# rajan-dubey8/camouflage-multimodal

Measured on AMD Instinct MI355X. Metric: images/sec fwd+bwd (fusion model train step: fwd + loss + bwd + clip + AdamW), higher is better.
Workload: dtype bf16; 1 GPU; BASELINE configs[1] on the path that exists (SURVEY 8d): cross-attention fusion model, packed variable-Nr minibatch (Nr ~ real 303..530 histogram, mean 483), Nk=13 real KG rows, train mode dropout 0.3, random-init weights; batch_per_gpu=16, global_batch=16, rg_dim=128, hidden_dim=256, num_heads=8, parallelism=dp1, precision=bf16 MFMA operands, fp32 accumulate/optimizer

## Files before the change

camouflage_multimodal_amd/csrc/fused_rows.hip:

```cpp
#include "fused_rows.h"
#include "shadow_inl.h"
#include "gemm.h"
#include "mfma_inl.h"

namespace {

template <int NT, int KS, bool W_IS_A, int DEPTH, bool USE_ROT = true>
struct Stage {
  static constexpr int TOTAL = NT * KS;
  static constexpr int D = DEPTH < TOTAL ? DEPTH : TOTAL;
  static_assert(!USE_ROT || (KS & (KS - 1)) == 0, "rotated k order: power-of-two k steps");
  u32x4 buf[D];
  const u32x4* wp; int rot;
  __device__ __forceinline__ int keff(int ks) const { return USE_ROT ? ((ks + rot) & (KS - 1)) : ks; }
  __device__ __forceinline__ const u32x4* wptr(int i) const { return wp + 64 * (keff(i / NT) * NT + (i % NT)); }
  __device__ __forceinline__ void prefetch(const u32x4* __restrict__ wp_, int rot_) {
    wp = wp_; rot = rot_;
#pragma unroll
    for (int i = 0; i < D; ++i) buf[i] = *wptr(i);
  }
  __device__ __forceinline__ void run(const char* act, f32x16 (&acc)[NT]) {
    run_f([&](int ks) { return *reinterpret_cast<const bf16x8*>(act + 32 * ks); }, acc);
  }
  template <class F>
// ... 31 lines not shown
__global__ __launch_bounds__(256) void shadow_kernel(const ShadowBatch sb, int total_chunks) {
  const int gid = blockIdx.x * 256 + threadIdx.x;
  for (int zi = 0; zi < sb.nzero; ++zi) {
    u32x4* z = static_cast<u32x4*>(sb.zero_ptr[zi]);
    const size_t n16 = sb.zero_bytes[zi] >> 4;
    for (size_t i = gid; i < n16; i += (size_t)gridDim.x * 256) z[i] = u32x4{0u, 0u, 0u, 0u};
  }
  if (gid >= total_chunks) return;
  int ji = 0;
#pragma unroll
  for (int i = 1; i < SHADOW_MAXJ; ++i)
    if (i < sb.n && gid >= sb.j[i].chunk_begin) ji = i;
  shadow_chunk(sb.j[ji], gid - sb.j[ji].chunk_begin);
}

constexpr int F_BUFR = 32 * PX, F_BUFQ = F_BUFR + 32 * PR, F_LDS = F_BUFQ + 32 * PQ;

template <int DEPTH, bool ROT>
__global__ __launch_bounds__(256, 2) void front_kernel(const FrontArgs a) {
  extern __shared__ __attribute__((aligned(16))) char smem[];
  const FrontStream& S = a.s[(int)blockIdx.x >= a.s[1].tile_begin ? 1 : 0];
  const int tid = threadIdx.x, lane = tid & 63, l31 = lane & 31, h = lane >> 5;
  const int w = __builtin_amdgcn_readfirstlane(tid >> 6);
  const int row0 = ((int)blockIdx.x - S.tile_begin) * 32;
  const int nrows = min(32, S.M - row0);
  char* bufX = smem; char* bufR = smem + F_BUFR; char* bufQ = smem + F_BUFQ;
  const int rot = ROT ? (int)(blockIdx.x >> 3) : 0;
  stamp(a.stamps, 0);
  Stage<2, 8, true, DEPTH> st0;
  st0.prefetch(reinterpret_cast<const u32x4*>(S.W0) + (size_t)w * (8 * 2 * 64) + lane, rot);
  {
    const int r = tid >> 3, c = tid & 7;
    const float4* src = reinterpret_cast<const float4*>(S.X + (size_t)(row0 + min(r, nrows - 1)) * 128 + 16 * c);
    float4 v0 = src[0], v1 = src[1], v2 = src[2], v3 = src[3];
    if (r >= nrows) { v0 = v1 = v2 = v3 = make_float4(0.f, 0.f, 0.f, 0.f); }
    *reinterpret_cast<u32x4*>(bufX + r * PX + 32 * c) = u32x4{pack2(v0.x, v0.y), pack2(v0.z, v0.w), pack2(v1.x, v1.y), pack2(v1.z, v1.w)};
    *reinterpret_cast<u32x4*>(bufX + r * PX + 32 * c + 16) = u32x4{pack2(v2.x, v2.y), pack2(v2.z, v2.w), pack2(v3.x, v3.y), pack2(v3.z, v3.w)};
  }
  __syncthreads();
  Stage<6, 16, true, DEPTH> st1;
  {
    f32x16 acc[2] = {zero16(), zero16()};
    st0.run(bufX + l31 * PX + 16 * h, acc);
    st1.prefetch(reinterpret_cast<const u32x4*>(S.W1) + (size_t)w * (16 * 6 * 64) + lane, rot);
#pragma unroll
    for (int t = 0; t < 2; ++t)
#pragma unroll
      for (int g = 0; g < 4; ++g) {
        const int c0 = 64 * w + 32 * t + 8 * g + 4 * h;
        const float4 bv = *reinterpret_cast<const float4*>(S.b0 + c0);
        *reinterpret_cast<u32x2*>(bufR + l31 * PR + 2 * c0) =
            u32x2{pack2(acc[t][4 * g] + bv.x, acc[t][4 * g + 1] + bv.y), pack2(acc[t][4 * g + 2] + bv.z, acc[t][4 * g + 3] + bv.w)};
      }
  }
  __syncthreads();
  stamp(a.stamps, 1);
  {
    f32x16 acc[6];
#pragma unroll
    for (int t = 0; t < 6; ++t) acc[t] = zero16();
    st1.run(bufR + l31 * PR + 16 * h, acc);
#pragma unroll
    for (int t = 0; t < 6; ++t) {
      const int tg = 6 * w + t;
      const float* bias = tg < 8 ? S.bq + 32 * tg : S.bkv + 32 * (tg - 8);
      const float sc = tg < 8 ? a.qscale : 1.0f;
#pragma unroll
      for (int g = 0; g < 4; ++g) {
        const int c = 8 * g + 4 * h;
        const float4 bv = *reinterpret_cast<const float4*>(bias + c);
        *reinterpret_cast<u32x2*>(bufQ + l31 * PQ + 2 * (32 * tg + c)) =
            u32x2{pack2((acc[t][4 * g] + bv.x) * sc, (acc[t][4 * g + 1] + bv.y) * sc),
                  pack2((acc[t][4 * g + 2] + bv.z) * sc, (acc[t][4 * g + 3] + bv.w) * sc)};
      }
    }
  }
  __syncthreads();
  stamp(a.stamps, 2);
  copy_out<5>(bufQ, PQ, 0, S.Q16, 256, row0, nrows);
  copy_out<6>(bufQ, PQ, 512, S.KV16, 512, row0, nrows);
  copy_out<5>(bufR, PR, 0, S.R16, 256, row0, nrows);
  if (a.save) copy_out<4>(bufX, PX, 0, S.X16, 128, row0, nrows);
  for (int zi = 0; zi < a.nzero; ++zi) {
    u32x4* z = static_cast<u32x4*>(a.zero_ptr[zi]);
    const unsigned n16 = a.zero_bytes[zi] >> 4;
    for (unsigned i = blockIdx.x * 256 + tid; i < n16; i += gridDim.x * 256) z[i] = u32x4{0u, 0u, 0u, 0u};
  }
  stamp(a.stamps, 3);
}

constexpr int PK = 528;
constexpr int PVC = 192;
constexpr int PT = 260;
constexpr int B_VS = 16 * PK;
template <int OCC> struct BackL;
template <> struct BackL<2> { static constexpr int XH = 0, O = 32 * PT * 4, Y = O + 32 * PR, RED = Y + 32 * PR, LDS = RED + 1024; };
template <> struct BackL<3> { static constexpr int Y = 0, XH = 32 * PR, O = 2 * 32 * PR, RED = O + 32 * PR, LDS = RED + 1024; };
constexpr int B_LDS = BackL<2>::LDS;
static_assert(BackL<3>::O >= 4 * 32 * 192 && BackL<3>::O >= 8448 + 9216 && BackL<2>::O >= 4 * 32 * 192, "attention scratch inside region A");

__device__ __forceinline__ void attn_rg_tile(const BackArgs& a, char* smem, char* bufO, int b, size_t row0, int nrows, int w, int lane) {
  const int tid = threadIdx.x, l31 = lane & 31, h = lane >> 5, Nk = a.Nk;
  char* Ks = smem; char* Vs = smem + B_VS;
  for (int c = tid; c < 16 * 64; c += 256) {
    const int j = c >> 6, ch = c & 63;
    u32x4 v = u32x4{0u, 0u, 0u, 0u};
    if (j < Nk) v = *reinterpret_cast<const u32x4*>(a.KV16 + ((size_t)b * Nk + j) * 512 + 8 * ch);
    if (ch < 32) *reinterpret_cast<u32x4*>(Ks + j * PK + 16 * ch) = v;
    else         *reinterpret_cast<u32x4*>(Vs + j * PV + 16 * (ch - 32)) = v;
  }
  const us16* qrow = a.Q16 + (row0 + min(l31, nrows - 1)) * 256 + 64 * w + 8 * h;
  bf16x8 qf[2][2];
#pragma unroll
  for (int hd = 0; hd < 2; ++hd)
#pragma unroll
    for (int s = 0; s < 2; ++s) qf[hd][s] = as_frag(*reinterpret_cast<const u32x4*>(qrow + 32 * hd + 16 * s));
  __syncthreads();
  const bool dodrop = a.drop.p > 0.f;
  const int q4 = (lane >> 2) & 3, p4 = lane & 3, g1 = (lane >> 4) & 1;
#pragma unroll
  for (int hd = 0; hd < 2; ++hd) {
    const int head = 2 * w + hd;
// ... 201 lines not shown
  const int w = __builtin_amdgcn_readfirstlane(tid >> 6);
  const int nkg = a.B * a.max_splits;
  const int vid = (int)blockIdx.x < a.lead_tiles ? nkg + (int)blockIdx.x : ((int)blockIdx.x < a.lead_tiles + nkg ? (int)blockIdx.x - a.lead_tiles : (int)blockIdx.x);
  const bool kg = vid < nkg;
  int rot = ROT ? (int)(blockIdx.x >> 3) : 0;
  using L = BackL<OCC>;
  char* bufO = smem + L::O; char* bufY = smem + L::Y;
  float* red = reinterpret_cast<float*>(smem + L::RED);
  float* tile32 = reinterpret_cast<float*>(smem);
  int b; size_t rowg0; int nrows; float inv_n;
  stamp(a.stamps, 0);
  const BackStream& S = a.s[kg ? 1 : 0];
  Stage<2, 16, true, DEPTH> sto;
  Stage<4, 16, false, DEPTH> stf;
  if (!kg) sto.prefetch(reinterpret_cast<const u32x4*>(S.Wo) + (size_t)w * (16 * 2 * 64) + lane, rot);
  if (kg) {
    b = vid / a.max_splits;
    const int sp = vid - b * a.max_splits;
    if (ROT) rot = b;
    const int nsplit = (a.off[b + 1] - a.off[b] + SPLIT_ROWS - 1) / SPLIT_ROWS;
    if (sp >= nsplit) return;
    attn_kg_split(a, smem, b, sp, w, lane);
    stamp(a.stamps, 4);
    asm volatile("s_waitcnt vmcnt(0)" ::: "memory");
    __syncthreads();
    int* flag = reinterpret_cast<int*>(red);
    if (tid == 0) flag[0] = __hip_atomic_fetch_add(a.tickets + b, 1, __ATOMIC_RELAXED, __HIP_MEMORY_SCOPE_AGENT);
    __syncthreads();
    stamp(a.stamps, 5);
    if (flag[0] != nsplit - 1) return;
    if (tid == 0) {
      __builtin_amdgcn_fence(__ATOMIC_ACQUIRE, "agent");
      asm volatile("s_waitcnt vmcnt(0)" ::: "memory");
    }
    for (int c = tid; c < 32 * PR / 16; c += 256) reinterpret_cast<u32x4*>(bufO)[c] = u32x4{0u, 0u, 0u, 0u};
    __syncthreads();
    sto.prefetch(reinterpret_cast<const u32x4*>(S.Wo) + (size_t)w * (16 * 2 * 64) + lane, rot);
    attn_kg_combine(a, smem, bufO, b, nsplit);
    stamp(a.stamps, 6);
    rowg0 = (size_t)b * a.Nk; nrows = a.Nk; inv_n = 1.0f / (float)a.Nk;
  } else {
    const int4 td = a.tile_desc[vid - nkg];
    if (td.x < 0) return;
    b = td.x; rowg0 = td.y; nrows = td.z; inv_n = __int_as_float(td.w);
    attn_rg_tile(a, smem, bufO, b, rowg0, nrows, w, lane);
  }
  __syncthreads();
  stamp(a.stamps, 1);

  const size_t rrow = rowg0 + min(l31, nrows - 1);
  float u[32];
  float rstd_keep = 0.f;
  {
    f32x16 acc[2] = {zero16(), zero16()};
    sto.run(bufO + l31 * PR + 16 * h, acc);
    stf.prefetch(reinterpret_cast<const u32x4*>(S.W1) + (size_t)w * (16 * 4 * 64) + lane, rot);
    float part = 0.f;
#pragma unroll
    for (int t = 0; t < 2; ++t)
#pragma unroll
      for (int g = 0; g < 4; ++g) {
        const int c0 = 64 * w + 32 * t + 8 * g + 4 * h;
        const float4 bv = *reinterpret_cast<const float4*>(S.bo + c0);
        const u32x2 rv = *reinterpret_cast<const u32x2*>(S.R16 + rrow * 256 + c0);
        float* o = u + 16 * t + 4 * g;
        o[0] = acc[t][4 * g] + bv.x + bf_lo(rv.x); o[1] = acc[t][4 * g + 1] + bv.y + bf_hi(rv.x);
        o[2] = acc[t][4 * g + 2] + bv.z + bf_lo(rv.y); o[3] = acc[t][4 * g + 3] + bv.w + bf_hi(rv.y);
        part += (o[0] + o[1]) + (o[2] + o[3]);
      }
    auto row_total = [&](float p, int slot) {
      p += __shfl_xor(p, 32, 64);
      if (h == 0) red[slot * 128 + w * 32 + l31] = p;
      __syncthreads();
      return (red[slot * 128 + l31] + red[slot * 128 + 32 + l31]) + (red[slot * 128 + 64 + l31] + red[slot * 128 + 96 + l31]);
    };
    const float mean = row_total(part, 0) * (1.0f / 256.0f);
    float sq = 0.f;
#pragma unroll
    for (int i = 0; i < 32; ++i) { u[i] -= mean; sq = fmaf(u[i], u[i], sq); }
    const float rstd = 1.0f / sqrtf(row_total(sq, 1) * (1.0f / 256.0f) + 1e-5f);
    rstd_keep = rstd;
    const bool rok = l31 < nrows;
#pragma unroll
    for (int t = 0; t < 2; ++t) {
      float ys[16];
#pragma unroll
      for (int g = 0; g < 4; ++g) {
        const int c0 = 64 * w + 32 * t + 8 * g + 4 * h;
        const float4 gm = *reinterpret_cast<const float4*>(S.ln_g + c0), bt = *reinterpret_cast<const float4*>(S.ln_b + c0);
        float* o = u + 16 * t + 4 * g;
        const float x0 = o[0] * rstd, x1 = o[1] * rstd, x2 = o[2] * rstd, x3 = o[3] * rstd;
        const float4 y = make_float4(x0 * gm.x + bt.x, x1 * gm.y + bt.y, x2 * gm.z + bt.z, x3 * gm.w + bt.w);
        *reinterpret_cast<u32x2*>(bufY + l31 * PR + 2 * c0) = u32x2{pack2(y.x, y.y), pack2(y.z, y.w)};
        if constexpr (OCC == 3) {
          ys[4 * g] = rok ? y.x : 0.f; ys[4 * g + 1] = rok ? y.y : 0.f; ys[4 * g + 2] = rok ? y.z : 0.f; ys[4 * g + 3] = rok ? y.w : 0.f;
          if (a.save) *reinterpret_cast<u32x2*>(smem + L::XH + l31 * PR + 2 * c0) = u32x2{pack2(x0, x1), pack2(x2, x3)};
        } else {
          *reinterpret_cast<float4*>(tile32 + l31 * PT + c0) = y;
          o[0] = x0; o[1] = x1; o[2] = x2; o[3] = x3;
        }
      }
      if constexpr (OCC == 2) continue;
#pragma unroll
      for (int st = 0; st < 4; ++st) {
// ... 3 lines not shown
        for (int i = 0; i < n; ++i) {
          const float send = up ? ys[i] : ys[i + n];
          const float keep = up ? ys[i + n] : ys[i];
          ys[i] = keep + __shfl_xor(send, m, 64);
        }
      }
      const float tot = ys[0] + __shfl_xor(ys[0], 1, 64);
      if ((l31 & 1) == 0) {
        const int i16 = (l31 >> 1) & 15;
        atomicAdd(S.Ymean + (size_t)b * 256 + 64 * w + 32 * t + 8 * (i16 >> 2) + 4 * h + (i16 & 3), tot * inv_n);
      }
    }
  }
  __syncthreads();
  stamp(a.stamps, 2);
  if constexpr (OCC == 2) {
    float sum = 0.f;
    for (int r = 0; r < nrows; ++r) sum += tile32[r * PT + tid];
    atomicAdd(S.Ymean + (size_t)b * 256 + tid, sum * inv_n);
  }

  {
    f32x16 acc[4] = {zero16(), zero16(), zero16(), zero16()};
    stf.run(bufY + l31 * PR + 16 * h, acc);
    const bool dodrop = a.drop.p > 0.f;
#pragma unroll
    for (int t = 0; t < 4; ++t) {
      const int f = 128 * w + 32 * t + l31;
      const float bias = S.b1[f];
      float colsum = 0.f;
      uint32_t wlo = 0u, whi = 0u;
#pragma unroll
      for (int i = 0; i < 16; ++i) {
        if (8 * (i >> 2) >= nrows) continue;
        const int row = acc_row(i, h);
        float v = fmaxf(acc[t][i] + bias, 0.f);
        if (dodrop) v *= drop_mult(a.drop, S.site_ffn, (uint32_t)(rowg0 + row) * 512u + (uint32_t)f);
        if (row >= nrows) v = 0.f;
        colsum += v;
        if (a.save) {
          const unsigned long long bal = __ballot(v > 0.f);
          SET_LANE(wlo, (uint32_t)bal, i); SET_LANE(whi, (uint32_t)(bal >> 32), i);
        }
      }
// ... 17 lines not shown
        for (int g = 0; g < 4; ++g) {
          const float* o = u + 16 * t + 4 * g;
          *reinterpret_cast<u32x2*>(bufXH + l31 * PR + 2 * (64 * w + 32 * t + 8 * g + 4 * h)) = u32x2{pack2(o[0], o[1]), pack2(o[2], o[3])};
        }
      __syncthreads();
    }
    copy_out<5>(bufXH, PR, 0, S.XH16, 256, rowg0, nrows);
    copy_out<5>(bufO, PR, 0, S.O16, 256, rowg0, nrows);
    copy_out<5>(bufY, PR, 0, S.Y16, 256, rowg0, nrows);
  }
  stamp(a.stamps, 3);
}


constexpr int W_GTAB = 0, W_BUFDU = 1024, W_KS = W_BUFDU + 32 * PR, W_VS = W_KS + 16 * PK, W_BUFDO = W_VS + 16 * PK,
              W_IMGS = W_BUFDO + 32 * PR, W_RED = W_IMGS + 16384, W_LDS = W_RED + 1024;
static_assert(32 * PR + 16384 == 32 * PT * 4, "the fp32 column-sum tile aliases [bufdO | images]");

__device__ __forceinline__ void tail_wg_tile(const TailWgArgs& g, int tile, float* dys, unsigned long long* stamps) {
  stamp(stamps, 0);
  int pi = 0;
  for (int i = 1; i < g.n; ++i) if (tile >= g.p[i].tile_begin) pi = i;
  const TailWgProd& P = g.p[pi];
  const int tid = threadIdx.x, B = g.B, ncb = P.cols >> 8, lt = tile - P.tile_begin, rb = lt / ncb;
  const int r0 = 16 * rb, c = 256 * (lt - rb * ncb) + tid;
  float xv[16], acc[16];
#pragma unroll
  for (int b = 0; b < 16; ++b) xv[b] = b < B ? P.x[(size_t)b * P.ld_x + c] : 0.f;
  const float dv = tid < B * 16 ? P.dy[(size_t)(tid >> 4) * P.ld_dy + r0 + (tid & 15)] : 0.f;
#pragma unroll
  for (int r = 0; r < 16; ++r) acc[r] = P.dW[(size_t)(r0 + r) * P.cols + c];
// ... 83 lines not shown
    const int4 td = a.tile_desc[blockIdx.x];
    if (td.x < 0) return;
    b = td.x; rowg0 = td.y; nrows = td.z; inv_n = __int_as_float(td.w);
  }
  const Bwd1Stream& S = a.s[kg ? 1 : 0];
  us16* gtab = reinterpret_cast<us16*>(smem + W_GTAB);
  char* bufdU = smem + W_BUFDU; char* bufQ = bufdU;
  char* Ks = smem + W_KS; char* Vs = smem + W_VS; char* bufdO = smem + W_BUFDO; char* imgs = smem + W_IMGS + w * 4096;
  float* red = reinterpret_cast<float*>(smem + W_RED);
  float* tile32 = reinterpret_cast<float*>(smem + W_BUFDO);
  stamp(a.stamps, 0);
  Stage<2, 32, true, DEPTH, false> st1;
  st1.prefetch(reinterpret_cast<const u32x4*>(S.W1T) + (size_t)w * (32 * 2 * 64) + lane, 0);
  const size_t vrow = rowg0 + min(l31, nrows - 1);
  const bool rok = l31 < nrows;
  {
    const float gs = inv_n * a.drop.scale;
    for (int f = tid; f < 512; f += 256) gtab[f] = f2bf(S.dHm[(size_t)b * S.ld_dHm + f] * gs);
  }
  u32x4 mw[4];
#pragma unroll
  for (int i = 0; i < 4; ++i) mw[i] = reinterpret_cast<const u32x4*>(S.mask + vrow * 16)[i];
  u32x4 qreg[4];
  if (!kg) {
#pragma unroll
    for (int i = 0; i < 4; ++i) {
      const int id = tid + 256 * i;
      qreg[i] = *reinterpret_cast<const u32x4*>(a.Q16 + (rowg0 + min(id >> 5, nrows - 1)) * 256 + 8 * (id & 31));
    }
    for (int c = tid; c < 16 * 64; c += 256) {
      const int j = c >> 6, ch = c & 63;
      u32x4 v = u32x4{0u, 0u, 0u, 0u};
      if (j < a.Nk) v = *reinterpret_cast<const u32x4*>(a.KV16 + ((size_t)b * a.Nk + j) * 512 + 8 * ch);
      if (ch < 32) *reinterpret_cast<u32x4*>(Ks + j * PK + 16 * ch) = v;
      else         *reinterpret_cast<u32x4*>(Vs + j * PK + 16 * (ch - 32)) = v;
    }
  }
  __syncthreads();
  Stage<2, 16, true, DEPTH> st2;
  f32x16 acc1[2] = {zero16(), zero16()};
  st1.run_f([&](int ks) {
    const uint32_t word = mw[ks >> 3][(ks >> 1) & 3];
    const uint32_t bits = (word >> (16 * (ks & 1))) >> (8 * h);
    const u32x4 g = *reinterpret_cast<const u32x4*>(smem + W_GTAB + 2 * (16 * ks + 8 * h));
    u32x4 fr;
#pragma unroll
    for (int d = 0; d < 4; ++d)
      fr[d] = (((bits >> (2 * d)) & 1u) ? (g[d] & 0xFFFFu) : 0u) | (((bits >> (2 * d + 1)) & 1u) ? (g[d] & 0xFFFF0000u) : 0u);
    return as_frag(fr);
  }, acc1);
  st2.prefetch(reinterpret_cast<const u32x4*>(S.WoT) + (size_t)w * (16 * 2 * 64) + lane, rot);
  stamp(a.stamps, 1);
  {
    float gg[32], xh[32];
    float s1 = 0.f, s2 = 0.f;
#pragma unroll
    for (int t = 0; t < 2; ++t)
#pragma unroll
      for (int g = 0; g < 4; ++g) {
        const int c0 = 64 * w + 32 * t + 8 * g + 4 * h;
        const float4 dc = *reinterpret_cast<const float4*>(S.dcomb + (size_t)b * S.ld_dcomb + c0);
        const float4 gm = *reinterpret_cast<const float4*>(S.ln_g + c0);
        const u32x2 xv = *reinterpret_cast<const u32x2*>(S.XH16 + vrow * 256 + c0);
        float* G = gg + 16 * t + 4 * g; float* X = xh + 16 * t + 4 * g;
        X[0] = bf_lo(xv.x); X[1] = bf_hi(xv.x); X[2] = bf_lo(xv.y); X[3] = bf_hi(xv.y);
        const float d0 = fmaf(dc.x, inv_n, acc1[t][4 * g]), d1 = fmaf(dc.y, inv_n, acc1[t][4 * g + 1]);
        const float d2 = fmaf(dc.z, inv_n, acc1[t][4 * g + 2]), d3 = fmaf(dc.w, inv_n, acc1[t][4 * g + 3]);
        *reinterpret_cast<float4*>(tile32 + l31 * PT + c0) = make_float4(d0 * X[0], d1 * X[1], d2 * X[2], d3 * X[3]);
        acc1[t][4 * g] = d0; acc1[t][4 * g + 1] = d1; acc1[t][4 * g + 2] = d2; acc1[t][4 * g + 3] = d3;
        G[0] = d0 * gm.x; G[1] = d1 * gm.y; G[2] = d2 * gm.z; G[3] = d3 * gm.w;
#pragma unroll
        for (int i = 0; i < 4; ++i) { s1 += G[i]; s2 = fmaf(G[i], X[i], s2); }
      }
    auto row_total = [&](float p, int slot) {
      p += __shfl_xor(p, 32, 64);
      if (h == 0) red[slot * 128 + w * 32 + l31] = p;
      __syncthreads();
      return (red[slot * 128 + l31] + red[slot * 128 + 32 + l31]) + (red[slot * 128 + 64 + l31] + red[slot * 128 + 96 + l31]);
    };
    const float m1 = row_total(s1, 0) * (1.0f / 256.0f);
    const float m2 = row_total(s2, 1) * (1.0f / 256.0f);
    {
      float sum = 0.f;
      for (int r = 0; r < nrows; ++r) sum += tile32[r * PT + tid];
      if (a.slabs & 1) a.slabLN[(size_t)blockIdx.x * 512 + tid] = sum;
      else atomicAdd(S.dgamma + tid, sum);
    }
    const float rstd = S.rstd[vrow];
#pragma unroll
    for (int t = 0; t < 2; ++t)
#pragma unroll
      for (int g = 0; g < 4; ++g) {
        const int c0 = 64 * w + 32 * t + 8 * g + 4 * h;
        const float* G = gg + 16 * t + 4 * g; const float* X = xh + 16 * t + 4 * g;
        float du[4];
#pragma unroll
        for (int i = 0; i < 4; ++i) du[i] = rok ? (G[i] - m1 - X[i] * m2) * rstd : 0.f;
        *reinterpret_cast<u32x2*>(bufdU + l31 * PR + 2 * c0) = u32x2{pack2(du[0], du[1]), pack2(du[2], du[3])};
      }
    __syncthreads();
#pragma unroll
    for (int t = 0; t < 2; ++t)
#pragma unroll
      for (int g = 0; g < 4; ++g) {
        const int c0 = 64 * w + 32 * t + 8 * g + 4 * h;
        *reinterpret_cast<float4*>(tile32 + l31 * PT + c0) = make_float4(acc1[t][4 * g], acc1[t][4 * g + 1], acc1[t][4 * g + 2], acc1[t][4 * g + 3]);
      }
    __syncthreads();
    {
      float sum = 0.f;
      for (int r = 0; r < nrows; ++r) sum += tile32[r * PT + tid];
      if (a.slabs & 1) a.slabLN[(size_t)blockIdx.x * 512 + 256 + tid] = sum;
      else atomicAdd(S.dbeta + tid, sum);
    }
  }
  stamp(a.stamps, 2);
  f32x16 acc2[2] = {zero16(), zero16()};
  st2.run(bufdU + l31 * PR + 16 * h, acc2);
  copy_out<5>(bufdU, PR, 0, S.dU16, 256, rowg0, nrows);
  if (kg) {
#pragma unroll
    for (int t = 0; t < 2; ++t) {
      float dot = 0.f;
#pragma unroll
      for (int g = 0; g < 4; ++g) {
        const int c0 = 64 * w + 32 * t + 8 * g + 4 * h;
        const u32x2 ov = *reinterpret_cast<const u32x2*>(a.O2_16 + vrow * 256 + c0);
        dot = fmaf(acc2[t][4 * g], bf_lo(ov.x), dot); dot = fmaf(acc2[t][4 * g + 1], bf_hi(ov.x), dot);
        dot = fmaf(acc2[t][4 * g + 2], bf_lo(ov.y), dot); dot = fmaf(acc2[t][4 * g + 3], bf_hi(ov.y), dot);
        if (rok) *reinterpret_cast<u32x2*>(a.dO2_16 + (rowg0 + l31) * 256 + c0) =
            u32x2{pack2(acc2[t][4 * g], acc2[t][4 * g + 1]), pack2(acc2[t][4 * g + 2], acc2[t][4 * g + 3])};
      }
      dot += __shfl_xor(dot, 32, 64);
      if (h == 0 && rok) a.delta2[((size_t)b * 8 + 2 * w + t) * 16 + l31] = dot;
    }
    stamp(a.stamps, 3);
    return;
  }
  __syncthreads();
#pragma unroll
  for (int i = 0; i < 4; ++i) { const int id = tid + 256 * i; *reinterpret_cast<u32x4*>(bufQ + (id >> 5) * PR + 16 * (id & 31)) = qreg[i]; }
#pragma unroll
// ... 130 lines not shown
  char* Q2s = smem + X_Q2S; char* dO2s = smem + X_DO2S; float* tabs = reinterpret_cast<float*>(smem + X_TABS);
  char* bufT = smem + X_BUFT; char* imgs = smem + X_IMGS;
  int* flag = reinterpret_cast<int*>(smem + X_RED);
  const int xb = (int)blockIdx.x - a.B - a.rg_tiles_max, xearly = (a.kg_split - 1) * a.B;
  if (xb >= xearly) { ln_slab_sum(a, xb - xearly); return; }
  stamp(a.stamps, 0);
  const bool early = (int)blockIdx.x < a.B || xb >= 0;
  int b;
  if (early) {
    b = xb >= 0 ? xb % a.B : (int)blockIdx.x;
    const int kq = xb >= 0 ? 1 + xb / a.B : 0;
    const int r_lo = a.kg_split > 1 ? min(4 * kq, Nk) : 0, r_hi = a.kg_split > 1 ? min(4 * kq + 4, Nk) : Nk;
    const size_t krow0 = (size_t)b * Nk;
    Stage<2, 32, true, DEPTH, false> se;
    se.prefetch(reinterpret_cast<const u32x4*>(a.WcKgT) + (size_t)w * (48 * 2 * 64) + 64 * (16 * 2) + lane, 0);
    const int t0 = a.tile_off[b], t1 = a.tile_off[b + 1];
    for (int c = tid; c < 32 * 64; c += 256) {
      const int j = c >> 6, ch = c & 63;
      u32x4 v = u32x4{0u, 0u, 0u, 0u};
      if (j >= r_lo && j < r_hi) {
        float4 x0, x1;
        if (a.slabs & 2) {
          x0 = x1 = make_float4(0.f, 0.f, 0.f, 0.f);
          const float* src = a.slabKV + (size_t)j * 512 + 8 * ch;
          for (int tb = t0; tb < t1; tb += SLAB_TILES) {
            float4 p0[SLAB_TILES], p1[SLAB_TILES];
#pragma unroll
            for (int u = 0; u < SLAB_TILES; ++u) {
              const float* s = src + (size_t)min(tb + u, t1 - 1) * Nk * 512;
              p0[u] = *reinterpret_cast<const float4*>(s); p1[u] = *reinterpret_cast<const float4*>(s + 4);
// ... 15 lines not shown
      }
      *reinterpret_cast<u32x4*>(bufT + j * PQ + 512 + 16 * ch) = v;
    }
    __syncthreads();
    f32x16 acc[2] = {zero16(), zero16()};
    se.run(bufT + l31 * PQ + 512 + 16 * h, acc);
    copy_out<6>(bufT + r_lo * PQ, PQ, 512, a.dQKVkg16 + 256, 768, krow0 + r_lo, r_hi - r_lo);
    if (a.kg_defer) {
      us16* const dGp16 = reinterpret_cast<us16*>(a.dGpart);
      if (l31 >= r_lo && l31 < r_hi) {
#pragma unroll
        for (int t = 0; t < 2; ++t)
#pragma unroll
          for (int g = 0; g < 4; ++g) {
            const int c0 = 64 * w + 32 * t + 8 * g + 4 * h;
            const u32x2 uv = *reinterpret_cast<const u32x2*>(a.dU2_16 + (krow0 + l31) * 256 + c0);
            *reinterpret_cast<u32x2*>(dGp16 + (krow0 + l31) * 256 + c0) =
                u32x2{pack2(acc[t][4 * g] + bf_lo(uv.x), acc[t][4 * g + 1] + bf_hi(uv.x)), pack2(acc[t][4 * g + 2] + bf_lo(uv.y), acc[t][4 * g + 3] + bf_hi(uv.y))};
          }
      }
      if (b == a.B - 1 && kq == 0) {
        const size_t tk = (size_t)a.B * Nk, n16 = (((tk + 127) & ~size_t(127)) - tk) * 32;
        for (size_t c = tid; c < n16; c += 256) *(reinterpret_cast<u32x4*>(dGp16 + tk * 256) + c) = u32x4{0u, 0u, 0u, 0u};
      }
    } else if (l31 >= r_lo && l31 < r_hi) {
#pragma unroll
      for (int t = 0; t < 2; ++t)
#pragma unroll
        for (int g = 0; g < 4; ++g) {
          const int c0 = 64 * w + 32 * t + 8 * g + 4 * h;
          const u32x2 uv = *reinterpret_cast<const u32x2*>(a.dU2_16 + (krow0 + l31) * 256 + c0);
          float* dst = a.dGpart + (krow0 + l31) * 256 + c0;
          __hip_atomic_store(dst, acc[t][4 * g] + bf_lo(uv.x), __ATOMIC_RELAXED, __HIP_MEMORY_SCOPE_AGENT);
          __hip_atomic_store(dst + 1, acc[t][4 * g + 1] + bf_hi(uv.x), __ATOMIC_RELAXED, __HIP_MEMORY_SCOPE_AGENT);
          __hip_atomic_store(dst + 2, acc[t][4 * g + 2] + bf_lo(uv.y), __ATOMIC_RELAXED, __HIP_MEMORY_SCOPE_AGENT);
          __hip_atomic_store(dst + 3, acc[t][4 * g + 3] + bf_hi(uv.y), __ATOMIC_RELAXED, __HIP_MEMORY_SCOPE_AGENT);
        }
    }
  } else {
  const int4 td = a.tile_desc[(int)blockIdx.x - a.B];
  if (td.x < 0) return;
  b = td.x;
  const size_t rowg0 = td.y;
  const int nrows = td.z;
  const bool rok = l31 < nrows;
  const size_t vrow = rowg0 + min(l31, nrows - 1);
  Stage<2, 48, true, DEPTH, false> sr;
  sr.prefetch(reinterpret_cast<const u32x4*>(a.WcRgT) + (size_t)w * (48 * 2 * 64) + lane, 0);
  for (int c = tid; c < 16 * 32; c += 256) {
    const int j = c >> 5, ch = c & 31;
    u32x4 q = u32x4{0u, 0u, 0u, 0u}, o = q;
    if (j < Nk) {
      q = *reinterpret_cast<const u32x4*>(a.Q2_16 + ((size_t)b * Nk + j) * 256 + 8 * ch);
      o = *reinterpret_cast<const u32x4*>(a.dO2_16 + ((size_t)b * Nk + j) * 256 + 8 * ch);
    }
    *reinterpret_cast<u32x4*>(Q2s + j * PK + 16 * ch) = q;
    *reinterpret_cast<u32x4*>(dO2s + j * PK + 16 * ch) = o;
  }
  if (tid < 128) {
    const int j = tid & 15;
    const size_t o = (size_t)b * 128 + tid;
    const bool ok = j < Nk;
    tabs[tid] = ok ? a.lse2[2 * o] : 0.f;
    tabs[128 + tid] = ok ? 1.0f / a.lse2[2 * o + 1] : 0.f;
    tabs[256 + tid] = ok ? a.delta2[o] : 0.f;
  }
  u32x4 dqreg[4];
#pragma unroll
  for (int i = 0; i < 4; ++i) {
    const int id = tid + 256 * i;
    const size_t r = rowg0 + min(id >> 5, nrows - 1);
    *reinterpret_cast<u32x4*>(bufT + (id >> 5) * PQ + 16 * (id & 31)) = *reinterpret_cast<const u32x4*>(a.KV2_16 + r * 512 + 8 * (id & 31));
    dqreg[i] = *reinterpret_cast<const u32x4*>(a.dQKV16 + r * 768 + 8 * (id & 31));
  }
  bf16x8 kf[2][2], vf[2][2];
  {
    const us16* kp = a.KV2_16 + vrow * 512 + 64 * w + 8 * h;
#pragma unroll
    for (int t = 0; t < 2; ++t)
#pragma unroll
      for (int s = 0; s < 2; ++s) {
        kf[t][s] = as_frag(*reinterpret_cast<const u32x4*>(kp + 32 * t + 16 * s));
        vf[t][s] = as_frag(*reinterpret_cast<const u32x4*>(kp + 256 + 32 * t + 16 * s));
      }
  }
  __syncthreads();
  const bool dodrop = a.drop.p > 0.f;
  const int q4 = (lane >> 2) & 3, p4 = lane & 3, g1 = (lane >> 4) & 1;
#pragma unroll
// ... 47 lines not shown
  __syncthreads();
  stamp(a.stamps, 1);
#pragma unroll
  for (int i = 0; i < 4; ++i) { const int id = tid + 256 * i; *reinterpret_cast<u32x4*>(bufT + (id >> 5) * PQ + 16 * (id & 31)) = dqreg[i]; }
  __syncthreads();
  {
    f32x16 acc[2] = {zero16(), zero16()};
    sr.run(bufT + l31 * PQ + 16 * h, acc);
    copy_out<6>(bufT, PQ, 512, a.dQKV16 + 256, 768, rowg0, nrows);
    if (rok) {
#pragma unroll
      for (int t = 0; t < 2; ++t)
#pragma unroll
        for (int g = 0; g < 4; ++g) {
          const int c0 = 64 * w + 32 * t + 8 * g + 4 * h;
          const u32x2 uv = *reinterpret_cast<const u32x2*>(a.dU16 + (rowg0 + l31) * 256 + c0);
          *reinterpret_cast<u32x2*>(a.dR16 + (rowg0 + l31) * 256 + c0) =
              u32x2{pack2(acc[t][4 * g] + bf_lo(uv.x), acc[t][4 * g + 1] + bf_hi(uv.x)), pack2(acc[t][4 * g + 2] + bf_lo(uv.y), acc[t][4 * g + 3] + bf_hi(uv.y))};
        }
    }
  }
  stamp(a.stamps, 2);
  }
  if (a.kg_defer) {
    if (early) { stamp(a.stamps, 1); stamp(a.stamps, 2); }
    stamp(a.stamps, 3);
    return;
  }
  asm volatile("s_waitcnt vmcnt(0)" ::: "memory");
  __syncthreads();
  if (tid == 0) flag[0] = __hip_atomic_fetch_add(a.tickets + b, 1, __ATOMIC_RELAXED, __HIP_MEMORY_SCOPE_AGENT);
// ... 11 lines not shown
    const int j = c >> 5, ch = c & 31;
    u32x4 v = u32x4{0u, 0u, 0u, 0u};
    if (j < Nk) {
      const float* src = a.dQ2acc + (krow0 + j) * 256 + 8 * ch;
      const float4 x0 = *reinterpret_cast<const float4*>(src), x1 = *reinterpret_cast<const float4*>(src + 4);
      v = u32x4{pack2(x0.x, x0.y), pack2(x0.z, x0.w), pack2(x1.x, x1.y), pack2(x1.z, x1.w)};
    }
    *reinterpret_cast<u32x4*>(bufT + j * PQ + 16 * ch) = v;
  }
  __syncthreads();
  {
    f32x16 acc[2] = {zero16(), zero16()};
    sg.run(bufT + l31 * PQ + 16 * h, acc);
    copy_out<5>(bufT, PQ, 0, a.dQKVkg16, 768, krow0, Nk);
    if (l31 < Nk) {
#pragma unroll
      for (int t = 0; t < 2; ++t)
#pragma unroll
        for (int g = 0; g < 4; ++g) {
          const int c0 = 64 * w + 32 * t + 8 * g + 4 * h;
          const float4 pv = *reinterpret_cast<const float4*>(a.dGpart + (krow0 + l31) * 256 + c0);
          *reinterpret_cast<u32x2*>(a.dG16 + (krow0 + l31) * 256 + c0) =
              u32x2{pack2(acc[t][4 * g] + pv.x, acc[t][4 * g + 1] + pv.y), pack2(acc[t][4 * g + 2] + pv.z, acc[t][4 * g + 3] + pv.w)};
        }
    }
  }
  stamp(a.stamps, 3);
}


template <int DEPTH, bool ROT>
__global__ __launch_bounds__(256, 2) void bwd2p_kernel(const Bwd2Args a) {
  extern __shared__ __attribute__((aligned(16))) char smem[];
  const int tid = threadIdx.x, lane = tid & 63, l31 = lane & 31, h = lane >> 5;
  const int w = __builtin_amdgcn_readfirstlane(tid >> 6);
  const int Nk = a.Nk;
// ... 302 lines not shown
```

Baseline: 101,700 images/s.

## Hoist global loads early and stage biases/params in LDS across fused kernels

Bias and LayerNorm parameter vectors are loaded once per block into new LDS tables instead of being re-read from global memory in the epilogues. Residual, XH, O2, dU and dGpart loads are issued into registers before the GEMM and attention phases so their latency overlaps compute. K/V staging loops are unrolled into batched loads followed by stores. Atomic reductions for Ymean and dgamma/dbeta are deferred until after the next GEMM so they leave the critical path. The cost is extra LDS per block and higher register pressure, which could lower occupancy.

```diff
diff --git a/camouflage_multimodal_amd/csrc/fused_rows.hip b/camouflage_multimodal_amd/csrc/fused_rows.hip
--- a/camouflage_multimodal_amd/csrc/fused_rows.hip
+++ b/camouflage_multimodal_amd/csrc/fused_rows.hip
@@ -69,7 +69,7 @@
   shadow_chunk(sb.j[ji], gid - sb.j[ji].chunk_begin);
 }
 
-constexpr int F_BUFR = 32 * PX, F_BUFQ = F_BUFR + 32 * PR, F_LDS = F_BUFQ + 32 * PQ;
+constexpr int F_BUFR = 32 * PX, F_BUFQ = F_BUFR + 32 * PR, F_PTAB = F_BUFQ + 32 * PQ, F_LDS = F_PTAB + 4096;
 
 template <int DEPTH, bool ROT>
 __global__ __launch_bounds__(256, 2) void front_kernel(const FrontArgs a) {
@@ -84,10 +84,13 @@
   stamp(a.stamps, 0);
   Stage<2, 8, true, DEPTH> st0;
   st0.prefetch(reinterpret_cast<const u32x4*>(S.W0) + (size_t)w * (8 * 2 * 64) + lane, rot);
+  float* ptab = reinterpret_cast<float*>(smem + F_PTAB);
   {
     const int r = tid >> 3, c = tid & 7;
     const float4* src = reinterpret_cast<const float4*>(S.X + (size_t)(row0 + min(r, nrows - 1)) * 128 + 16 * c);
     float4 v0 = src[0], v1 = src[1], v2 = src[2], v3 = src[3];
+    const float p0 = S.b0[tid], p1 = S.bq[tid], p2 = S.bkv[tid], p3 = S.bkv[256 + tid];
+    ptab[tid] = p0; ptab[256 + tid] = p1; ptab[512 + tid] = p2; ptab[768 + tid] = p3;
     if (r >= nrows) { v0 = v1 = v2 = v3 = make_float4(0.f, 0.f, 0.f, 0.f); }
     *reinterpret_cast<u32x4*>(bufX + r * PX + 32 * c) = u32x4{pack2(v0.x, v0.y), pack2(v0.z, v0.w), pack2(v1.x, v1.y), pack2(v1.z, v1.w)};
     *reinterpret_cast<u32x4*>(bufX + r * PX + 32 * c + 16) = u32x4{pack2(v2.x, v2.y), pack2(v2.z, v2.w), pack2(v3.x, v3.y), pack2(v3.z, v3.w)};
@@ -103,7 +106,7 @@
 #pragma unroll
       for (int g = 0; g < 4; ++g) {
         const int c0 = 64 * w + 32 * t + 8 * g + 4 * h;
-        const float4 bv = *reinterpret_cast<const float4*>(S.b0 + c0);
+        const float4 bv = *reinterpret_cast<const float4*>(ptab + c0);
         *reinterpret_cast<u32x2*>(bufR + l31 * PR + 2 * c0) =
             u32x2{pack2(acc[t][4 * g] + bv.x, acc[t][4 * g + 1] + bv.y), pack2(acc[t][4 * g + 2] + bv.z, acc[t][4 * g + 3] + bv.w)};
       }
@@ -118,7 +121,7 @@
 #pragma unroll
     for (int t = 0; t < 6; ++t) {
       const int tg = 6 * w + t;
-      const float* bias = tg < 8 ? S.bq + 32 * tg : S.bkv + 32 * (tg - 8);
+      const float* bias = ptab + 256 + 32 * tg;
       const float sc = tg < 8 ? a.qscale : 1.0f;
 #pragma unroll
       for (int g = 0; g < 4; ++g) {
@@ -149,7 +152,7 @@
 constexpr int PT = 260;
 constexpr int B_VS = 16 * PK;
 template <int OCC> struct BackL;
-template <> struct BackL<2> { static constexpr int XH = 0, O = 32 * PT * 4, Y = O + 32 * PR, RED = Y + 32 * PR, LDS = RED + 1024; };
+template <> struct BackL<2> { static constexpr int XH = 0, O = 32 * PT * 4, Y = O + 32 * PR, RED = Y + 32 * PR, PTAB = RED + 1024, LDS = PTAB + 5120; };
 template <> struct BackL<3> { static constexpr int Y = 0, XH = 32 * PR, O = 2 * 32 * PR, RED = O + 32 * PR, LDS = RED + 1024; };
 constexpr int B_LDS = BackL<2>::LDS;
 static_assert(BackL<3>::O >= 4 * 32 * 192 && BackL<3>::O >= 8448 + 9216 && BackL<2>::O >= 4 * 32 * 192, "attention scratch inside region A");
@@ -157,10 +160,16 @@
 __device__ __forceinline__ void attn_rg_tile(const BackArgs& a, char* smem, char* bufO, int b, size_t row0, int nrows, int w, int lane) {
   const int tid = threadIdx.x, l31 = lane & 31, h = lane >> 5, Nk = a.Nk;
   char* Ks = smem; char* Vs = smem + B_VS;
-  for (int c = tid; c < 16 * 64; c += 256) {
-    const int j = c >> 6, ch = c & 63;
-    u32x4 v = u32x4{0u, 0u, 0u, 0u};
-    if (j < Nk) v = *reinterpret_cast<const u32x4*>(a.KV16 + ((size_t)b * Nk + j) * 512 + 8 * ch);
+  u32x4 kv[4];
+#pragma unroll
+  for (int i = 0; i < 4; ++i) {
+    const int c = tid + 256 * i;
+    kv[i] = *reinterpret_cast<const u32x4*>(a.KV16 + ((size_t)b * Nk + min(c >> 6, Nk - 1)) * 512 + 8 * (c & 63));
+  }
+#pragma unroll
+  for (int i = 0; i < 4; ++i) {
+    const int c = tid + 256 * i, j = c >> 6, ch = c & 63;
+    const u32x4 v = j < Nk ? kv[i] : u32x4{0u, 0u, 0u, 0u};
     if (ch < 32) *reinterpret_cast<u32x4*>(Ks + j * PK + 16 * ch) = v;
     else         *reinterpret_cast<u32x4*>(Vs + j * PV + 16 * (ch - 32)) = v;
   }
@@ -392,6 +401,18 @@
   Stage<2, 16, true, DEPTH> sto;
   Stage<4, 16, false, DEPTH> stf;
   if (!kg) sto.prefetch(reinterpret_cast<const u32x4*>(S.Wo) + (size_t)w * (16 * 2 * 64) + lane, rot);
+  float* ptab = reinterpret_cast<float*>(smem + BackL<2>::PTAB);
+  float pt[5];
+  u32x2 rres[2][4];
+  auto load_early = [&](size_t row) {
+    if constexpr (OCC == 2) {
+      pt[0] = S.bo[tid]; pt[1] = S.ln_g[tid]; pt[2] = S.ln_b[tid]; pt[3] = S.b1[tid]; pt[4] = S.b1[256 + tid];
+#pragma unroll
+      for (int t = 0; t < 2; ++t)
+#pragma unroll
+        for (int g = 0; g < 4; ++g) rres[t][g] = *reinterpret_cast<const u32x2*>(S.R16 + row * 256 + 64 * w + 32 * t + 8 * g + 4 * h);
+    }
+  };
   if (kg) {
     b = vid / a.max_splits;
     const int sp = vid - b * a.max_splits;
@@ -414,6 +435,7 @@
     for (int c = tid; c < 32 * PR / 16; c += 256) reinterpret_cast<u32x4*>(bufO)[c] = u32x4{0u, 0u, 0u, 0u};
     __syncthreads();
     sto.prefetch(reinterpret_cast<const u32x4*>(S.Wo) + (size_t)w * (16 * 2 * 64) + lane, rot);
+    load_early((size_t)b * a.Nk + min(l31, a.Nk - 1));
     attn_kg_combine(a, smem, bufO, b, nsplit);
     stamp(a.stamps, 6);
     rowg0 = (size_t)b * a.Nk; nrows = a.Nk; inv_n = 1.0f / (float)a.Nk;
@@ -421,10 +443,19 @@
     const int4 td = a.tile_desc[vid - nkg];
     if (td.x < 0) return;
     b = td.x; rowg0 = td.y; nrows = td.z; inv_n = __int_as_float(td.w);
+    load_early(rowg0 + min(l31, nrows - 1));
     attn_rg_tile(a, smem, bufO, b, rowg0, nrows, w, lane);
   }
+  if constexpr (OCC == 2) {
+#pragma unroll
+    for (int i = 0; i < 5; ++i) ptab[256 * i + tid] = pt[i];
+  }
   __syncthreads();
   stamp(a.stamps, 1);
+  auto pvec = [&](const float* g, int at, int c) {
+    if constexpr (OCC == 2) return *reinterpret_cast<const float4*>(ptab + at + c);
+    else return *reinterpret_cast<const float4*>(g + c);
+  };
 
   const size_t rrow = rowg0 + min(l31, nrows - 1);
   float u[32];
@@ -439,8 +470,10 @@
 #pragma unroll
       for (int g = 0; g < 4; ++g) {
         const int c0 = 64 * w + 32 * t + 8 * g + 4 * h;
-        const float4 bv = *reinterpret_cast<const float4*>(S.bo + c0);
-        const u32x2 rv = *reinterpret_cast<const u32x2*>(S.R16 + rrow * 256 + c0);
+        const float4 bv = pvec(S.bo, 0, c0);
+        u32x2 rv;
+        if constexpr (OCC == 2) rv = rres[t][g];
+        else rv = *reinterpret_cast<const u32x2*>(S.R16 + rrow * 256 + c0);
         float* o = u + 16 * t + 4 * g;
         o[0] = acc[t][4 * g] + bv.x + bf_lo(rv.x); o[1] = acc[t][4 * g + 1] + bv.y + bf_hi(rv.x);
         o[2] = acc[t][4 * g + 2] + bv.z + bf_lo(rv.y); o[3] = acc[t][4 * g + 3] + bv.w + bf_hi(rv.y);
@@ -465,7 +498,7 @@
 #pragma unroll
       for (int g = 0; g < 4; ++g) {
         const int c0 = 64 * w + 32 * t + 8 * g + 4 * h;
-        const float4 gm = *reinterpret_cast<const float4*>(S.ln_g + c0), bt = *reinterpret_cast<const float4*>(S.ln_b + c0);
+        const float4 gm = pvec(S.ln_g, 256, c0), bt = pvec(S.ln_b, 512, c0);
         float* o = u + 16 * t + 4 * g;
         const float x0 = o[0] * rstd, x1 = o[1] * rstd, x2 = o[2] * rstd, x3 = o[3] * rstd;
         const float4 y = make_float4(x0 * gm.x + bt.x, x1 * gm.y + bt.y, x2 * gm.z + bt.z, x3 * gm.w + bt.w);
@@ -499,20 +532,24 @@
   }
   __syncthreads();
   stamp(a.stamps, 2);
+  float ymean_keep = 0.f;
   if constexpr (OCC == 2) {
     float sum = 0.f;
     for (int r = 0; r < nrows; ++r) sum += tile32[r * PT + tid];
-    atomicAdd(S.Ymean + (size_t)b * 256 + tid, sum * inv_n);
+    ymean_keep = sum * inv_n;
   }
 
   {
     f32x16 acc[4] = {zero16(), zero16(), zero16(), zero16()};
     stf.run(bufY + l31 * PR + 16 * h, acc);
+    if constexpr (OCC == 2) atomicAdd(S.Ymean + (size_t)b * 256 + tid, ymean_keep);
     const bool dodrop = a.drop.p > 0.f;
 #pragma unroll
     for (int t = 0; t < 4; ++t) {
       const int f = 128 * w + 32 * t + l31;
-      const float bias = S.b1[f];
+      float bias;
+      if constexpr (OCC == 2) bias = ptab[768 + f];
+      else bias = S.b1[f];
       float colsum = 0.f;
       uint32_t wlo = 0u, whi = 0u;
 #pragma unroll
@@ -560,7 +597,8 @@
 
 
 constexpr int W_GTAB = 0, W_BUFDU = 1024, W_KS = W_BUFDU + 32 * PR, W_VS = W_KS + 16 * PK, W_BUFDO = W_VS + 16 * PK,
-              W_IMGS = W_BUFDO + 32 * PR, W_RED = W_IMGS + 16384, W_LDS = W_RED + 1024;
+              W_IMGS = W_BUFDO + 32 * PR, W_RED = W_IMGS + 16384, W_PTAB = W_RED + 1024, W_LDS = W_PTAB + 2048;
+static_assert(W_VS == W_KS + 16 * PK && 32 * PR == 2 * 16 * PK, "a KG block parks its O2 rows (32 x PR) in the two idle key | value images");
 static_assert(32 * PR + 16384 == 32 * PT * 4, "the fp32 column-sum tile aliases [bufdO | images]");
 
 __device__ __forceinline__ void tail_wg_tile(const TailWgArgs& g, int tile, float* dys, unsigned long long* stamps) {
@@ -674,10 +712,24 @@
   st1.prefetch(reinterpret_cast<const u32x4*>(S.W1T) + (size_t)w * (32 * 2 * 64) + lane, 0);
   const size_t vrow = rowg0 + min(l31, nrows - 1);
   const bool rok = l31 < nrows;
-  {
-    const float gs = inv_n * a.drop.scale;
-    for (int f = tid; f < 512; f += 256) gtab[f] = f2bf(S.dHm[(size_t)b * S.ld_dHm + f] * gs);
-  }
+  float* ptab = reinterpret_cast<float*>(smem + W_PTAB);
+  const float rstd = S.rstd[vrow];
+  const float ptv0 = S.dcomb[(size_t)b * S.ld_dcomb + tid], ptv1 = S.ln_g[tid];
+  u32x2 xv[2][4], ov[2][4];
+#pragma unroll
+  for (int t = 0; t < 2; ++t)
+#pragma unroll
+    for (int g = 0; g < 4; ++g) {
+      const int c0 = 64 * w + 32 * t + 8 * g + 4 * h;
+      xv[t][g] = *reinterpret_cast<const u32x2*>(S.XH16 + vrow * 256 + c0);
+    }
+  if (kg) {
+#pragma unroll
+    for (int t = 0; t < 2; ++t)
+#pragma unroll
+      for (int g = 0; g < 4; ++g) ov[t][g] = *reinterpret_cast<const u32x2*>(a.O2_16 + vrow * 256 + 64 * w + 32 * t + 8 * g + 4 * h);
+  }
+  const float dh0 = S.dHm[(size_t)b * S.ld_dHm + tid], dh1 = S.dHm[(size_t)b * S.ld_dHm + 256 + tid];
   u32x4 mw[4];
 #pragma unroll
   for (int i = 0; i < 4; ++i) mw[i] = reinterpret_cast<const u32x4*>(S.mask + vrow * 16)[i];
@@ -688,14 +740,33 @@
       const int id = tid + 256 * i;
       qreg[i] = *reinterpret_cast<const u32x4*>(a.Q16 + (rowg0 + min(id >> 5, nrows - 1)) * 256 + 8 * (id & 31));
     }
-    for (int c = tid; c < 16 * 64; c += 256) {
-      const int j = c >> 6, ch = c & 63;
-      u32x4 v = u32x4{0u, 0u, 0u, 0u};
-      if (j < a.Nk) v = *reinterpret_cast<const u32x4*>(a.KV16 + ((size_t)b * a.Nk + j) * 512 + 8 * ch);
+    u32x4 kv[4];
+#pragma unroll
+    for (int i = 0; i < 4; ++i) {
+      const int c = tid + 256 * i;
+      kv[i] = *reinterpret_cast<const u32x4*>(a.KV16 + ((size_t)b * a.Nk + min(c >> 6, a.Nk - 1)) * 512 + 8 * (c & 63));
+    }
+#pragma unroll
+    for (int i = 0; i < 4; ++i) {
+      const int c = tid + 256 * i, j = c >> 6, ch = c & 63;
+      const u32x4 v = j < a.Nk ? kv[i] : u32x4{0u, 0u, 0u, 0u};
       if (ch < 32) *reinterpret_cast<u32x4*>(Ks + j * PK + 16 * ch) = v;
       else         *reinterpret_cast<u32x4*>(Vs + j * PK + 16 * (ch - 32)) = v;
     }
   }
+  {
+    const float gs = inv_n * a.drop.scale;
+    gtab[tid] = f2bf(dh0 * gs); gtab[256 + tid] = f2bf(dh1 * gs);
+  }
+  ptab[tid] = ptv0; ptab[256 + tid] = ptv1;
+#pragma unroll
+  for (int t = 0; t < 2; ++t)
+#pragma unroll
+    for (int g = 0; g < 4; ++g) {
+      const int c0 = 64 * w + 32 * t + 8 * g + 4 * h;
+      *reinterpret_cast<u32x2*>(bufdU + l31 * PR + 2 * c0) = xv[t][g];
+      if (kg) *reinterpret_cast<u32x2*>(Ks + l31 * PR + 2 * c0) = ov[t][g];
+    }
   __syncthreads();
   Stage<2, 16, true, DEPTH> st2;
   f32x16 acc1[2] = {zero16(), zero16()};
@@ -711,6 +782,7 @@
   }, acc1);
   st2.prefetch(reinterpret_cast<const u32x4*>(S.WoT) + (size_t)w * (16 * 2 * 64) + lane, rot);
   stamp(a.stamps, 1);
+  float sum_g = 0.f, sum_b = 0.f;
   {
     float gg[32], xh[32];
     float s1 = 0.f, s2 = 0.f;
@@ -719,9 +791,9 @@
 #pragma unroll
       for (int g = 0; g < 4; ++g) {
         const int c0 = 64 * w + 32 * t + 8 * g + 4 * h;
-        const float4 dc = *reinterpret_cast<const float4*>(S.dcomb + (size_t)b * S.ld_dcomb + c0);
-        const float4 gm = *reinterpret_cast<const float4*>(S.ln_g + c0);
-        const u32x2 xv = *reinterpret_cast<const u32x2*>(S.XH16 + vrow * 256 + c0);
+        const float4 dc = *reinterpret_cast<const float4*>(ptab + c0);
+        const float4 gm = *reinterpret_cast<const float4*>(ptab + 256 + c0);
+        const u32x2 xv = *reinterpret_cast<const u32x2*>(bufdU + l31 * PR + 2 * c0);
         float* G = gg + 16 * t + 4 * g; float* X = xh + 16 * t + 4 * g;
         X[0] = bf_lo(xv.x); X[1] = bf_hi(xv.x); X[2] = bf_lo(xv.y); X[3] = bf_hi(xv.y);
         const float d0 = fmaf(dc.x, inv_n, acc1[t][4 * g]), d1 = fmaf(dc.y, inv_n, acc1[t][4 * g + 1]);
@@ -740,13 +812,7 @@
     };
     const float m1 = row_total(s1, 0) * (1.0f / 256.0f);
     const float m2 = row_total(s2, 1) * (1.0f / 256.0f);
-    {
-      float sum = 0.f;
-      for (int r = 0; r < nrows; ++r) sum += tile32[r * PT + tid];
-      if (a.slabs & 1) a.slabLN[(size_t)blockIdx.x * 512 + tid] = sum;
-      else atomicAdd(S.dgamma + tid, sum);
-    }
-    const float rstd = S.rstd[vrow];
+    for (int r = 0; r < nrows; ++r) sum_g += tile32[r * PT + tid];
 #pragma unroll
     for (int t = 0; t < 2; ++t)
 #pragma unroll
@@ -767,16 +833,18 @@
         *reinterpret_cast<float4*>(tile32 + l31 * PT + c0) = make_float4(acc1[t][4 * g], acc1[t][4 * g + 1], acc1[t][4 * g + 2], acc1[t][4 * g + 3]);
       }
     __syncthreads();
-    {
-      float sum = 0.f;
-      for (int r = 0; r < nrows; ++r) sum += tile32[r * PT + tid];
-      if (a.slabs & 1) a.slabLN[(size_t)blockIdx.x * 512 + 256 + tid] = sum;
-      else atomicAdd(S.dbeta + tid, sum);
-    }
+    for (int r = 0; r < nrows; ++r) sum_b += tile32[r * PT + tid];
   }
   stamp(a.stamps, 2);
   f32x16 acc2[2] = {zero16(), zero16()};
   st2.run(bufdU + l31 * PR + 16 * h, acc2);
+  if (a.slabs & 1) {
+    a.slabLN[(size_t)blockIdx.x * 512 + tid] = sum_g;
+    a.slabLN[(size_t)blockIdx.x * 512 + 256 + tid] = sum_b;
+  } else {
+    atomicAdd(S.dgamma + tid, sum_g);
+    atomicAdd(S.dbeta + tid, sum_b);
+  }
   copy_out<5>(bufdU, PR, 0, S.dU16, 256, rowg0, nrows);
   if (kg) {
 #pragma unroll
@@ -785,7 +853,7 @@
 #pragma unroll
       for (int g = 0; g < 4; ++g) {
         const int c0 = 64 * w + 32 * t + 8 * g + 4 * h;
-        const u32x2 ov = *reinterpret_cast<const u32x2*>(a.O2_16 + vrow * 256 + c0);
+        const u32x2 ov = *reinterpret_cast<const u32x2*>(Ks + l31 * PR + 2 * c0);
         dot = fmaf(acc2[t][4 * g], bf_lo(ov.x), dot); dot = fmaf(acc2[t][4 * g + 1], bf_hi(ov.x), dot);
         dot = fmaf(acc2[t][4 * g + 2], bf_lo(ov.y), dot); dot = fmaf(acc2[t][4 * g + 3], bf_hi(ov.y), dot);
         if (rok) *reinterpret_cast<u32x2*>(a.dO2_16 + (rowg0 + l31) * 256 + c0) =
@@ -946,6 +1014,11 @@
     const size_t krow0 = (size_t)b * Nk;
     Stage<2, 32, true, DEPTH, false> se;
     se.prefetch(reinterpret_cast<const u32x4*>(a.WcKgT) + (size_t)w * (48 * 2 * 64) + 64 * (16 * 2) + lane, 0);
+    u32x2 du2reg[2][4];
+#pragma unroll
+    for (int t = 0; t < 2; ++t)
+#pragma unroll
+      for (int g = 0; g < 4; ++g) du2reg[t][g] = *reinterpret_cast<const u32x2*>(a.dU2_16 + (krow0 + min(l31, Nk - 1)) * 256 + 64 * w + 32 * t + 8 * g + 4 * h);
     const int t0 = a.tile_off[b], t1 = a.tile_off[b + 1];
     for (int c = tid; c < 32 * 64; c += 256) {
       const int j = c >> 6, ch = c & 63;
@@ -991,7 +1064,7 @@
 #pragma unroll
           for (int g = 0; g < 4; ++g) {
             const int c0 = 64 * w + 32 * t + 8 * g + 4 * h;
-            const u32x2 uv = *reinterpret_cast<const u32x2*>(a.dU2_16 + (krow0 + l31) * 256 + c0);
+            const u32x2 uv = du2reg[t][g];
             *reinterpret_cast<u32x2*>(dGp16 + (krow0 + l31) * 256 + c0) =
                 u32x2{pack2(acc[t][4 * g] + bf_lo(uv.x), acc[t][4 * g + 1] + bf_hi(uv.x)), pack2(acc[t][4 * g + 2] + bf_lo(uv.y), acc[t][4 * g + 3] + bf_hi(uv.y))};
           }
@@ -1006,7 +1079,7 @@
 #pragma unroll
         for (int g = 0; g < 4; ++g) {
           const int c0 = 64 * w + 32 * t + 8 * g + 4 * h;
-          const u32x2 uv = *reinterpret_cast<const u32x2*>(a.dU2_16 + (krow0 + l31) * 256 + c0);
+          const u32x2 uv = du2reg[t][g];
           float* dst = a.dGpart + (krow0 + l31) * 256 + c0;
           __hip_atomic_store(dst, acc[t][4 * g] + bf_lo(uv.x), __ATOMIC_RELAXED, __HIP_MEMORY_SCOPE_AGENT);
           __hip_atomic_store(dst + 1, acc[t][4 * g + 1] + bf_hi(uv.x), __ATOMIC_RELAXED, __HIP_MEMORY_SCOPE_AGENT);
@@ -1024,23 +1097,30 @@
   const size_t vrow = rowg0 + min(l31, nrows - 1);
   Stage<2, 48, true, DEPTH, false> sr;
   sr.prefetch(reinterpret_cast<const u32x4*>(a.WcRgT) + (size_t)w * (48 * 2 * 64) + lane, 0);
-  for (int c = tid; c < 16 * 32; c += 256) {
-    const int j = c >> 5, ch = c & 31;
-    u32x4 q = u32x4{0u, 0u, 0u, 0u}, o = q;
-    if (j < Nk) {
-      q = *reinterpret_cast<const u32x4*>(a.Q2_16 + ((size_t)b * Nk + j) * 256 + 8 * ch);
-      o = *reinterpret_cast<const u32x4*>(a.dO2_16 + ((size_t)b * Nk + j) * 256 + 8 * ch);
-    }
-    *reinterpret_cast<u32x4*>(Q2s + j * PK + 16 * ch) = q;
-    *reinterpret_cast<u32x4*>(dO2s + j * PK + 16 * ch) = o;
-  }
-  if (tid < 128) {
-    const int j = tid & 15;
-    const size_t o = (size_t)b * 128 + tid;
-    const bool ok = j < Nk;
-    tabs[tid] = ok ? a.lse2[2 * o] : 0.f;
-    tabs[128 + tid] = ok ? 1.0f / a.lse2[2 * o + 1] : 0.f;
-    tabs[256 + tid] = ok ? a.delta2[o] : 0.f;
+  {
+    u32x4 q[2], o[2];
+#pragma unroll
+    for (int i = 0; i < 2; ++i) {
+      const int c = tid + 256 * i;
+      const size_t r = (size_t)b * Nk + min(c >> 5, Nk - 1);
+      q[i] = *reinterpret_cast<const u32x4*>(a.Q2_16 + r * 256 + 8 * (c & 31));
+      o[i] = *reinterpret_cast<const u32x4*>(a.dO2_16 + r * 256 + 8 * (c & 31));
+    }
+    const size_t lo = (size_t)b * 128 + (tid & 127);
+    const float2 ml = *reinterpret_cast<const float2*>(a.lse2 + 2 * lo);
+    const float d2 = a.delta2[lo];
+#pragma unroll
+    for (int i = 0; i < 2; ++i) {
+      const int c = tid + 256 * i, j = c >> 5, ch = c & 31;
+      *reinterpret_cast<u32x4*>(Q2s + j * PK + 16 * ch) = j < Nk ? q[i] : u32x4{0u, 0u, 0u, 0u};
+      *reinterpret_cast<u32x4*>(dO2s + j * PK + 16 * ch) = j < Nk ? o[i] : u32x4{0u, 0u, 0u, 0u};
+    }
+    if (tid < 128) {
+      const bool ok = (tid & 15) < Nk;
+      tabs[tid] = ok ? ml.x : 0.f;
+      tabs[128 + tid] = ok ? 1.0f / ml.y : 0.f;
+      tabs[256 + tid] = ok ? d2 : 0.f;
+    }
   }
   u32x4 dqreg[4];
 #pragma unroll
@@ -1050,6 +1130,11 @@
     *reinterpret_cast<u32x4*>(bufT + (id >> 5) * PQ + 16 * (id & 31)) = *reinterpret_cast<const u32x4*>(a.KV2_16 + r * 512 + 8 * (id & 31));
     dqreg[i] = *reinterpret_cast<const u32x4*>(a.dQKV16 + r * 768 + 8 * (id & 31));
   }
+  u32x2 dureg[2][4];
+#pragma unroll
+  for (int t = 0; t < 2; ++t)
+#pragma unroll
+    for (int g = 0; g < 4; ++g) dureg[t][g] = *reinterpret_cast<const u32x2*>(a.dU16 + vrow * 256 + 64 * w + 32 * t + 8 * g + 4 * h);
   bf16x8 kf[2][2], vf[2][2];
   {
     const us16* kp = a.KV2_16 + vrow * 512 + 64 * w + 8 * h;
@@ -1127,7 +1212,7 @@
 #pragma unroll
         for (int g = 0; g < 4; ++g) {
           const int c0 = 64 * w + 32 * t + 8 * g + 4 * h;
-          const u32x2 uv = *reinterpret_cast<const u32x2*>(a.dU16 + (rowg0 + l31) * 256 + c0);
+          const u32x2 uv = dureg[t][g];
           *reinterpret_cast<u32x2*>(a.dR16 + (rowg0 + l31) * 256 + c0) =
               u32x2{pack2(acc[t][4 * g] + bf_lo(uv.x), acc[t][4 * g + 1] + bf_hi(uv.x)), pack2(acc[t][4 * g + 2] + bf_lo(uv.y), acc[t][4 * g + 3] + bf_hi(uv.y))};
         }
@@ -1169,12 +1254,17 @@
     sg.run(bufT + l31 * PQ + 16 * h, acc);
     copy_out<5>(bufT, PQ, 0, a.dQKVkg16, 768, krow0, Nk);
     if (l31 < Nk) {
+      float4 pvs[2][4];
+#pragma unroll
+      for (int t = 0; t < 2; ++t)
+#pragma unroll
+        for (int g = 0; g < 4; ++g) pvs[t][g] = *reinterpret_cast<const float4*>(a.dGpart + (krow0 + l31) * 256 + 64 * w + 32 * t + 8 * g + 4 * h);
 #pragma unroll
       for (int t = 0; t < 2; ++t)
 #pragma unroll
         for (int g = 0; g < 4; ++g) {
           const int c0 = 64 * w + 32 * t + 8 * g + 4 * h;
-          const float4 pv = *reinterpret_cast<const float4*>(a.dGpart + (krow0 + l31) * 256 + c0);
+          const float4 pv = pvs[t][g];
           *reinterpret_cast<u32x2*>(a.dG16 + (krow0 + l31) * 256 + c0) =
               u32x2{pack2(acc[t][4 * g] + pv.x, acc[t][4 * g + 1] + pv.y), pack2(acc[t][4 * g + 2] + pv.z, acc[t][4 * g + 3] + pv.w)};
         }
```

After: 104,700 images/s (median of 6 runs). 3.0% higher.
